# YamaneKoyo/mri-to-speech

Measured on AMD Instinct MI355X. Metric: rtMRI frames/s end-to-end (256x256 frames -> 64-bin mel -> 11413 Hz wav), higher is better.
Workload: dtype bf16x3; 1 GPU; e2e rtMRI->wav, 64 clips x 30 frames per GPU at 256x256 (configs[3] per-GPU share); clips_per_gpu=64, frames_per_clip=30, global_batch_clips=64, hw=256, parallelism=dp1, chunk=1920

## Files before the change

mri-to-speech_amd/csrc/conv1d_halo.hip:

```cpp
#include <cstring>

#include "conv_igemm.hpp"
#include "kernels.hpp"
#include "prof.hpp"

namespace m2s {
namespace {

__device__ __attribute__((aligned(16))) uint4 g_h1_zero[4];

constexpr int H1_BM = 128;
constexpr int H1_HIST = 64;
constexpr int H1_ROWS = H1_BM + H1_HIST;
constexpr int H1_PLANE = H1_ROWS * 16;

template <int C>
constexpr int h1_stage() {
  return 2 * (C / 16) * 1024;
}
template <int C>
constexpr int h1_slots() {
  return C <= 64 ? 4 : 3;
}
template <int C>
// ... 134 lines not shown
    for (int nt = 0; nt < NTW; ++nt) {
      const int n4 = (ntb + nt) * 16 + 4 * g;
      const float4 bb = *reinterpret_cast<const float4*>(a.bias + n4);
      float v[4] = {acc[i][nt][0] + bb.x, acc[i][nt][1] + bb.y, acc[i][nt][2] + bb.z, acc[i][nt][3] + bb.w};
      auto apply_act = [&]() {
        if (a.act == ACT_LRELU) {
#pragma unroll
          for (int j = 0; j < 4; ++j) v[j] = v[j] > 0.f ? v[j] : v[j] * a.act_slope;
        }
      };
      if (!a.act_after_res) apply_act();
      if (Rs) {
        float r[4], rl[4];
        unpack_bf16x4(prh[i][nt], r);
        unpack_bf16x4(prl[i][nt], rl);
#pragma unroll
        for (int j = 0; j < 4; ++j) {
          r[j] += rl[j];
          if (a.res_unslope != 0.f) r[j] = r[j] > 0.f ? r[j] : r[j] * a.res_unslope;
          v[j] += r[j];
        }
      }
      if (a.accum) {
        float p[4], pl[4];
        unpack_bf16x4(pyh[i][nt], p);
        unpack_bf16x4(pyl[i][nt], pl);
#pragma unroll
        for (int j = 0; j < 4; ++j) v[j] = (p[j] + pl[j]) + v[j];
        if (a.accum == 2) {
#pragma unroll
          for (int j = 0; j < 4; ++j) v[j] = v[j] / a.accum_div;
        }
      }
      if (a.act_after_res) apply_act();
      uint2 hi, lo;
      split4(v, hi, lo);
      *reinterpret_cast<uint2*>(Y + orow + n4) = hi;
      *reinterpret_cast<uint2*>(Y + orow + a.cs_out + n4) = lo;
    }
  }
}

template <int C>
void launch_c(const ConvBatch& b, int n, int B, int L, hipStream_t s, double flops, double bytes) {
  allow_lds(reinterpret_cast<const void*>(&conv1d_halo_sp_kernel<C>));
  const int tiles = ceil_div(L, H1_BM);
  char name[48];
  snprintf(name, sizeof(name), "conv1d_halo_sp_kernel<%d>", C);
  ProfScope ps(name, flops, bytes, s);
  hipLaunchKernelGGL((conv1d_halo_sp_kernel<C>), dim3(B * tiles, 1, n), dim3(64 * h1_waves<C>()), h1_lds<C>(), s, b, tiles);
  M2S_HIP(hipGetLastError());
}

}

bool conv1d_halo_sp_supported(int C, int cs, int k, int dil) {
  return C == 64 && cs == C && k >= 1 && k <= 31 && dil >= 1 && (k - 1) * dil <= H1_HIST;
}
size_t conv1d_halo_frag_elems(int C, int k) { return (size_t)k * (C / 32) * 2 * C * 32; }

void launch_conv1d_halo_sp(const ConvArgs* as, int n, hipStream_t s, double flops, double bytes) {
  M2S_CHECK(n >= 1 && n <= CONV_BATCH, "conv1d_halo: 1..CONV_BATCH convs");
  const ConvArgs& a = as[0];
  ConvBatch b;
  std::memset(&b, 0, sizeof(b));
  for (int i = 0; i < n; ++i) {
    const ConvArgs& c = as[i];
    M2S_CHECK(c.kind == KIND_CONV1D && c.cs_in == a.cs_in && c.cs_out == a.cs_in && c.M == a.M && c.L_in == c.L_out &&
                  c.L_out == a.L_out && c.in_xform == IN_NONE && c.pad_left == (c.ntaps - 1) * c.dil &&
                  conv1d_halo_sp_supported(a.cs_in, c.cs_in, c.ntaps, c.dil),
              "conv1d_halo: causal 1-D convs of one shape, C = 64, (k - 1) d <= 64");
    M2S_CHECK(c.x && c.w && c.bias && c.y && c.y != c.x && c.y != c.res, "conv1d_halo: operand pointers");
    for (int j = 0; j < i; ++j) M2S_CHECK(as[j].y != c.y, "conv1d_halo: two convs write one output");
    b.a[i] = c;
  }
  const int L = a.L_out, B = a.M / L;
  M2S_CHECK(B * L == a.M && L > 0, "conv1d_halo: M = clips x L");
  M2S_CHECK((double)a.M * a.cs_in * 2 < 2147483647.0, "conv1d_halo: 32-bit offsets");
  launch_c<64>(b, n, B, L, s, flops, bytes);
}

}
```

mri-to-speech_amd/csrc/kernels.hpp:

```cpp
#pragma once

#include "m2s_common.hpp"

namespace m2s {

enum AsyncCode : unsigned { M2S_ASYNC_LSTM = 1u, M2S_ASYNC_WS = 2u };
struct AsyncReport {
  unsigned spin_max = 1u << 20;
  unsigned* err = nullptr;
};
__device__ __forceinline__ void report_async(unsigned* err, unsigned code, int lane) {
  if (err && lane == 0) __hip_atomic_store(err, code, __ATOMIC_RELAXED, __HIP_MEMORY_SCOPE_SYSTEM);
}

template <typename T>
void launch_stem(const float* frames, int N, int H, int W, int OH, int OW, int pad_t, int pad_l,
                 const float* w9, const float* bias, int cout, int cs_out, T* y, hipStream_t s);

int dw_pixel_blocks(int OH, int OW);
template <typename T>
void launch_dwconv(const T* x, int N, int IH, int IW, int OH, int OW, int stride, int pad_t, int pad_l,
                   int C, int cs, const float* w9, const float* bias, T* y, float* sums, hipStream_t s);

template <typename T>
void launch_se_mean(const float* psum, int N, int npb, int cs, float inv_count, T* mean, hipStream_t s);

bool ir_fused_supported(int OH, int OW, int cs_in, int cs_mid, bool split);
void launch_ir_pwdw(const void* x, int N, int cs_in, int kp, const void* wpw, const float* bpw, const void* wdw,
                    const float* bdw, int OH, int OW, int cs_mid, void* y, void* se_mean, bool split, double flops,
                    double bytes, hipStream_t s, bool f8_out = false, const void* x8 = nullptr,
                    const void* w8 = nullptr, const float* wsc = nullptr, int kp8 = 0);
void launch_rows_e4m3(const void* x, long rows, int cs, void* y8, int ld8, hipStream_t s);

bool se_gemm_f8_supported(int P, int cs_in, int cs_out);
void launch_se_gemm_f8(const void* x8, int M, int P, int cs_in, const void* w8, int kp, int n_pad, const float* wscale,
                       const float* bias, const void* gate, const void* res, void* y, int cs_out, hipStream_t s,
                       double flops, double bytes, void* y8 = nullptr, int ld8 = 0);

bool se_gemm_sp_supported(int P, int cs_in, int cs_out);
void launch_se_gemm_sp(const void* x, int M, int P, int cs_in, const void* w, int n_pad, const float* bias,
                       const void* gate, const void* res, void* y, int cs_out, hipStream_t s, double flops, double bytes);

bool se_ws_supported(int P, int cs_in, int cs_out);
void launch_se_ws(const void* x, int M, int P, int cs_in, const void* w, int n_pad, const float* bias, const void* gate,
                  const void* res, void* y, int cs_out, hipStream_t s, double flops, double bytes, AsyncReport rep = {},
                  bool x_f32 = false);

bool se_ws_f8_supported(int P, int cs_in, int cs_out);
void launch_se_ws_f8(const void* x8, int M, int P, int cs_in, const void* w8, int kp, int n_pad, const float* wscale,
                     const float* bias, const void* gate, const void* res, void* y, int cs_out, hipStream_t s, double flops,
                     double bytes, void* y8 = nullptr, int ld8 = 0, AsyncReport rep = {});

bool ir_ws_supported(int H, int W, int cs_in, int kp, int cs_mid);
bool ir_ws_s2_supported(int H, int W, int cs_in, int kp, int cs_mid, int OH, int OW, int pad_t, int pad_l);
void launch_ir_ws(const void* x, int N, int H, int W, int cs_in, int kp, int cs_mid, const void* wpw, const float* bpw,
                  const float* wdw, const float* bdw, void* y, void* se_mean, double flops, double bytes,
                  hipStream_t s, AsyncReport rep = {}, int stride = 1, int OH = 0, int OW = 0, int pad_t = 0,
                  int pad_l = 0, double spill = 0.0, bool fm32 = false);
int ir_s2band_bands(int OH);
bool ir_s2band_supported(int IH, int IW, int OH, int OW, int cs_in, int kp, int cs_mid);
void launch_ir_s2band(const void* x, int N, int IH, int IW, int cs_in, int kp, const void* wpw, const float* bpw,
                      const float* wdw, const float* bdw, int OH, int OW, int pad_t, int pad_l, int cs_mid, void* y,
                      float* psum, bool split, double flops, double bytes, hipStream_t s, bool f8_out = false);
bool ir_fused_s2_supported(int IH, int IW, int cs_in, int cs_mid, bool split);
void launch_ir_pwdw_s2(const void* x, int N, int cs_in, int kp, const void* wpw, const float* bpw, const void* wdw,
                       const float* bdw, int IH, int IW, int OH, int OW, int pad_t, int pad_l, int cs_mid, void* y,
                       void* se_mean, bool split, double flops, double bytes, hipStream_t s, bool f8_out = false,
                       const void* x8 = nullptr, const void* w8 = nullptr, const float* wsc = nullptr, int kp8 = 0);

bool conv1d_halo_sp_supported(int C, int cs, int k, int dil);
size_t conv1d_halo_frag_elems(int C, int k);
void launch_conv1d_halo_sp(const struct ConvArgs* a, int n, hipStream_t s, double flops, double bytes);
bool rb1_fused_supported(int C, int cs, int k, const int* dil, int np, int kp, bool split);
int rb1_frag_taps(int C, int k, bool split);
void launch_rb1_fused(const bf16_t* x, bf16_t* s, int B, int L, int C, int k, int np, const int* dil,
                      const bf16_t* const* w1, const float* const* b1, const bf16_t* const* w2,
                      const float* const* b2, int kp, int accum, float div, bool split, double flops, double bytes,
                      hipStream_t st);

void launch_stem_b0(const float* frames, int N, int H, int W, int OH, int OW, int pad_t, int pad_l, const float* w9,
                    const float* b9, const void* w0, const float* b0, int kp0, const void* w1, const float* b1,
                    int kp1, void* y, bool split, double flops, double bytes, hipStream_t s);

bool se_excite_supported(int rd, int kp2, int cs_mid);
void launch_se_excite(const void* mean, int N, int mid, int cs_mid, const void* w1, int kp1, const float* b1,
                      int rd, const void* w2, int kp2, const float* b2, void* gate, bool split, hipStream_t s);

bool er_fused_supported(int H, int W, int cin, int mid, int cout, int kp_exp, int kp_pwl);
void launch_er_fused(const bf16_t* x, int N, int H, int W, const bf16_t* wexp, const float* bexp, const bf16_t* wpwl,
                     const float* bpwl, bf16_t* y, double flops, double bytes, hipStream_t s);

bool er8_fused_supported(int H, int W, int cin, int mid, int cout);
void launch_er8_fused(const bf16_t* x, int N, int H, int W, const uint8_t* wexp, const float* sexp, const float* bexp,
                      const uint8_t* wpwl, const float* spwl, const float* bpwl, bf16_t* y, double flops, double bytes,
                      hipStream_t s, const uint8_t* x8 = nullptr, uint8_t* y8 = nullptr);

bool er2_fused_supported(int H, int W, int cs_in, int mid, int cout, int kp_exp, int kp_pwl);
int er2_stage_elems();
bool er8w_fused_supported(int H, int W, int cs_in, int mid, int cout);
size_t er8w_stream_bytes();
void launch_er8w_fused(const bf16_t* x, const uint8_t* x8, int N, int H, int W, const uint8_t* wst, const float* sexp,
                       const float* bexp, const float* spwl, const float* bpwl, bf16_t* y, uint8_t* y8, double flops,
                       double bytes, hipStream_t s);
void launch_er2_fused(const bf16_t* x, int N, int H, int W, const bf16_t* wst, const float* bexp, const float* bpwl,
                      bf16_t* y, double flops, double bytes, hipStream_t s);

bool er_sp_supported(int H, int W, int cs_in, int mid, int cs_out);
int er_sp_nt_stages(int cs_in, int mid, int cs_out, int* nt);
void launch_er_sp(const void* x, int N, int H, int W, int cs_in, int mid, int cs_out, const void* wst, const float* bexp,
                  const float* bpwl, void* y, double flops, double bytes, hipStream_t s, bool merged = true);

bool ers2_fused_supported(int OH, int OW, int cs_in, int mid, int cs_out, int kp_exp, int kp_pwl);
int ers2_exp_elems(int cs_in, int mid);
bool ers2_sp_supported(int OH, int OW, int cs_in, int mid, int cs_out);
void launch_ers2_sp(const void* x, int N, int H, int W, int OH, int OW, int pad_t, int pad_l, int cs_in, int mid,
                    int cs_out, const void* wexp, const float* bexp, const void* wpwl, const float* bpwl, void* y,
                    double flops, double bytes, hipStream_t s);
void launch_ers2_fused(const bf16_t* x, int N, int H, int W, int OH, int OW, int pad_t, int pad_l, int cs_in, int mid,
                       int cs_out, const bf16_t* wexp, const float* bexp, const bf16_t* wpwl, const float* bpwl,
                       bf16_t* y, double flops, double bytes, hipStream_t s, uint8_t* y8 = nullptr);

void launch_preprocess(const uint8_t* frames, int N, int H, int W, int channels, float* out, hipStream_t s);

template <typename T>
void launch_gap(const T* x, int N, int P, int C, int cs, float* feats, hipStream_t s);
// ... 78 lines not shown
```

mri-to-speech_amd/csrc/model.cpp:

```cpp
#include "model.hpp"

#include <algorithm>
#include <cmath>
#include <cstdlib>
#include <cstring>
#include <initializer_list>
#include <type_traits>
#include <utility>

#include "pack.hpp"
#include "prof.hpp"

namespace m2s {

void Arena::upload(int device) {
  M2S_HIP(hipSetDevice(device));
  M2S_HIP(hipMalloc(&dev_, host_.size() + 256));
  M2S_HIP(hipMemcpy(dev_, host_.data(), host_.size(), hipMemcpyHostToDevice));
  std::vector<uint8_t>().swap(host_);
}

Arena::~Arena() {
  if (dev_) (void)hipFree(dev_);
}
// ... 742 lines not shown
  a.y = b.pre;
  a.M = (int)N;
  a.kwave = 0;
  run_conv<float>(a, p_.lstm_ih, s);
  {
    ProfScope ps("lstm_window_table_kernel", 0.0, 4.0 * (5.0 * B + 2.0 * S), s);
    launch_lstm_window_table(b.tab, B, W, p.mean, p.max_windows, b.win, s);
  }
  const size_t plane = (size_t)S * H;
  {
    const double cells = p.active[0] + (p.mean ? 0.0 : (double)S);
    ProfScope ps("lstm_window_step0_kernel", 0.0, 4.0 * cells * H * (3.0 + 2.0), s);
    launch_lstm_window_step0(b.pre, b.win, S, !p.mean, split, b.hop[0], b.c, p.mean ? b.hf : (W == 1 ? b.hm : nullptr),
                             p.mean ? b.hf + (size_t)W * plane : b.hm + (size_t)p.R * H, s);
  }
  const float* wperm = static_cast<const float*>(arena_.ptr(p_.whh_win));
  for (int j = 1; j < W; ++j) {
    const void* hin = b.hop[(j - 1) & 1];
    void* hout = j + 1 < W ? b.hop[j & 1] : nullptr;
    float* hf = p.mean ? b.hf + (size_t)j * plane : (j == W - 1 ? b.hm : nullptr);
    ProfScope ps(split ? "lstm_window_step_kernel<split>" : "lstm_window_step_kernel<f32>",
                 (split ? 3.0 : 2.0) * 4.0 * H * H * p.active[j], 4.0 * dirs * 4 * H * H + 4.0 * p.active[j] * H * 8.0, s);
    launch_lstm_window_step(b.pre, wperm, b.win, S, j, dirs, split, hin, hout, b.c, hf, (long)((size_t)W * plane), s);
  }
  if (p.mean) {
    double contrib = 0.0;
    for (int j = 0; j < W; ++j) contrib += p.active[j];
    ProfScope ps("lstm_window_mean_kernel", contrib * H, 4.0 * H * (contrib + 2.0 * p.N), s);
    launch_lstm_window_mean(b.hf, b.tab, B, W, S, p.N, p.max_len, b.hm, s);
  }
  if (mel_norm) {
    StageTag head("head");
    ProfScope ps("mel_head_kernel", 2.0 * p.R * H * n_mels_, 4.0 * p.R * (2 * H + n_mels_), s);
    launch_mel_head(b.hm, (int)p.R, H, static_cast<const float*>(arena_.ptr(p_.head_wt)),
                    static_cast<const float*>(arena_.ptr(p_.head_b)), n_mels_, mel_norm, s);
  }
  if (y) launch_add2(b.hm, b.hm + (size_t)p.R * H, y, (long)((size_t)p.R * H), s);
}

void Acoustic::forward_windowed(const float* frames, const int* lengths, const int* context, int B, long N, int H,
                                int W, int window, int merge, float* mel_norm, Workspace& ws, hipStream_t s) {
  M2S_CHECK(lstm_window_supported(hidden_), "windowed: rnn_hidden must be 640");
  window_plan(lengths, context, B, N, window, merge);
  ragged_check_stream(s);
  float* feats = feats_buf(ws, (size_t)N);
  effnet(frames, (int)N, H, W, feats, -1, nullptr, nullptr, ws, s);
  bilstm_windowed(feats, lengths, context, B, N, window, merge, nullptr, mel_norm, ws, s);
}

Vocoder::Vocoder(const StateDict& sd, const m2s_hifigan_h& h, int dtype, int device)
    : h_(h), dtype_(dtype), device_(device) {
  for (auto [name, v] : std::initializer_list<std::pair<const char*, bool*>>{
           {"M2S_MRF_FUSED", &mrf_fused_}, {"M2S_MRF_BATCH", &mrf_batch_}, {"M2S_MRF_HALO", &mrf_halo_},
           {"M2S_F8_MRF64", &f8_mrf64_},   {"M2S_F8_MRF32", &f8_mrf32_}})
    env_flag(name, *v);
  pack_vocoder(sd, h, dtype, f8_mrf64_, f8_mrf32_, arena_, p_);
  arena_.upload(device);
  p_.pre.resolve(arena_);
  for (auto& u : p_.ups) u.resolve(arena_);
  for (auto& rb : p_.rbs) {
    for (auto& c : rb.c1) c.resolve(arena_);
    for (auto& c : rb.c2) c.resolve(arena_);
    for (size_t o : rb.f1_off) rb.f1.push_back(static_cast<const bf16_t*>(arena_.ptr(o)));
    for (size_t o : rb.f2_off) rb.f2.push_back(static_cast<const bf16_t*>(arena_.ptr(o)));
    for (size_t o : rb.h1_off) rb.h1.push_back(static_cast<const bf16_t*>(arena_.ptr(o)));
    for (size_t o : rb.h2_off) rb.h2.push_back(static_cast<const bf16_t*>(arena_.ptr(o)));
    for (auto* qv : {&rb.q1, &rb.q2})
      for (RB::F8& f : *qv) {
        f.wp = arena_.ptr(f.w);
        f.sp = static_cast<const float*>(arena_.ptr(f.s));
        f.bp = static_cast<const float*>(arena_.ptr(f.b));
      }
  }
}

size_t Vocoder::act_elems(int B, int T) const {
  size_t m = (size_t)B * T * chan_stride(h_.upsample_initial_channel);
  size_t L = T;
  for (int i = 0; i < h_.n_up; ++i) {
    L *= h_.upsample_rates[i];
    m = std::max(m, (size_t)B * L * chan_stride(h_.upsample_initial_channel >> (i + 1)));
  }
  return m;
}

void* Vocoder::mel_in(Workspace& ws, int B, int T) const {
  return ws.take<char>((size_t)B * T * chan_stride(h_.num_mels) * act_bytes(dtype_));
}

template <typename T>
Vocoder::GenBufs<T> Vocoder::gen_bufs(Workspace& ws, int B, int T_) const {
  const size_t n = act_elems(B, T_) * Elem<T>::R;
  GenBufs<T> g{};
  g.X = ws.take<T>(n);
  for (T*& h : g.Hb) h = ws.take<T>(n);
  g.T1 = ws.take<T>(n);
  g.S = ws.take<T>(n);
  if (dtype_ == M2S_DT_FP8) g.E8 = ws.take<T>(n);
  if (std::is_same<T, sp_t>::value)
    for (auto& bt : g.Bt)
      for (T*& q : bt) q = ws.take<T>(n);
  return g;
}

void Vocoder::gen_ws(Workspace& ws, int B, int T) const {
  dispatch_act(dtype_, [&](auto t) { gen_bufs<typename decltype(t)::type>(ws, B, T); });
}

size_t Vocoder::workspace_bytes(int B, int T) const {
// ... 134 lines not shown
}


size_t Vocoder::chunk_workspace_bytes(const int* lengths, const int* context, const int* hold, int B) const {
  long n = 0;
  for (int b = 0; lengths && b < B; ++b) n += lengths[b];
  const ChunkPlan p = chunk_plan(lengths, context, hold, B, n);
  return Workspace::bytes([&](Workspace& ws) {
    ragged_bufs(ws, B, p.d.Tmax, 5 + h_.n_up);
    gen_ws(ws, B, p.d.Tmax);
  });
}

void Vocoder::forward_chunk(const float* mel, const int* lengths, const int* context, const int* hold, int B, long N,
                            float* wav, Workspace& ws, hipStream_t s) {
  const ChunkPlan p = chunk_plan(lengths, context, hold, B, N);
  const int nm = h_.num_mels, cs = chan_stride(nm), T = p.d.Tmax;
  const RaggedBufs cb = ragged_bufs(ws, B, T, 5 + h_.n_up);
  rtab_.upload_ints(p.tab.data(), p.tab.size(), cb.tab, s);
  Cone cone{};
  for (int l = 0; l < h_.n_up; ++l) {
    cone.drop[l] = p.drop[l];
    cone.keep[l] = p.keep[l];
    cone.mask[l] = p.mask ? cb.tab + (size_t)(4 + l) * B : nullptr;
  }
  dispatch_act(dtype_, [&](auto t) {
    using A = typename decltype(t)::type;
    {
      StageTag tag("glue");
      ProfScope ps(tname<A>("ragged_glue_kernel"), 0.0, 4.0 * N * nm * 2, s);
      launch_ragged_glue<A>(mel, cb.tab, B, T, nm, nullptr, nullptr, nullptr, nullptr, static_cast<A*>(cb.ln_buf), cs,
                            s);
    }
    run_t<A>(cb.ln_buf, B, T, cb.wav_pad, ws, s, p.mask ? cb.tab : nullptr, p.crop ? &cone : nullptr);
  });
  StageTag tag("voc_post");
  ProfScope ps("chunk_wav_pack_kernel", 0.0, 2.0 * 4.0 * p.out_rows * p_.hop, s);
  const int* const emit = cb.tab + (size_t)2 * B;
  launch_chunk_wav_pack(cb.wav_pad, emit, emit + B, emit + (size_t)2 * B, B, p.t_final, p_.hop, wav, s);
}

constexpr int CONV_POST_TAPS = 7;

template <typename T>
void Vocoder::mrf_stage_batched(int i, const T* X, T* S, T* const (*Bt)[3], int B, int L, bool act_out,
                                hipStream_t s) {
  const int nk = h_.n_kernels, np = (int)p_.rbs[i * nk].dil.size();
  int ord[CONV_BATCH];
  for (int j = 0; j < nk; ++j) ord[j] = j;
  std::sort(ord, ord + nk, [&](int x, int y) { return p_.rbs[i * nk + x].c1[0].kp > p_.rbs[i * nk + y].c1[0].kp; });
  auto a_in = [&](int j, int p) -> const T* { return p == 0 ? X : Bt[j][1 + ((p - 1) & 1)]; };
  bool halo = mrf_halo_;
  for (int j = 0; j < nk; ++j) halo = halo && !p_.rbs[i * nk + j].h1.empty();
  auto launch_batch = [&](ConvArgs* cs, int n, double fl, double by) {
    if (halo)
      launch_conv1d_halo_sp(cs, n, s, fl, by);
    else
      launch_conv_gemm_batch(cs, n, s, fl, by);
  };
  for (int p = 0; p < np; ++p) {
    ConvArgs cs[CONV_BATCH];
    double fl = 0.0, by = 0.0, f, b;
    for (int jj = 0; jj < nk; ++jj) {
      const int j = ord[jj];
      const RB& rb = p_.rbs[i * nk + j];
      ConvArgs c = conv_args(rb.c1[p]);
      if (halo) c.w = rb.h1[p];
      c.x = a_in(j, p);
      c.y = Bt[j][0];
      c.L_in = c.L_out = L;
      c.M = B * L;
      c.act = ACT_LRELU;
      c.act_slope = 0.1f;
      conv_cost<T>(c, rb.c1[p], &f, &b);
      fl += f;
      by += b;
      cs[jj] = c;
    }
    launch_batch(cs, nk, fl, by);
    fl = by = 0.0;
    for (int jj = 0; jj < nk; ++jj) {
      const int j = p + 1 < np ? ord[jj] : jj;
      const RB& rb = p_.rbs[i * nk + j];
      ConvArgs c = conv_args(rb.c2[p]);
      if (halo) c.w = rb.h2[p];
      c.x = Bt[j][0];
      c.res = a_in(j, p);
      c.res_unslope = 10.f;
      c.L_in = c.L_out = L;
      c.M = B * L;
      if (p + 1 < np) {
        c.y = Bt[j][1 + (p & 1)];
        c.act = ACT_LRELU;
        c.act_slope = 0.1f;
        c.act_after_res = 1;
        conv_cost<T>(c, rb.c2[p], &f, &b);
        fl += f;
        by += b;
        cs[jj] = c;
      } else {
        c.y = S;
        c.accum = j == 0 ? 0 : (j == nk - 1 ? 2 : 1);
        c.accum_div = (float)nk;
        if (act_out && j == nk - 1) {
          c.act = ACT_LRELU;
          c.act_slope = 0.1f;
// ... 225 lines not shown
```

mri-to-speech_amd/csrc/model.hpp:

```cpp
#pragma once

#include <map>
#include <string>
#include <vector>

#include "../../include/m2s.h"
#include "conv_igemm.hpp"
#include "kernels.hpp"

namespace m2s {

struct HostTensor {
  const float* data = nullptr;
  std::vector<int64_t> shape;
  size_t numel() const {
    size_t n = 1;
    for (auto d : shape) n *= (size_t)d;
    return n;
  }
};
using StateDict = std::map<std::string, HostTensor>;
StateDict make_state_dict(const m2s_tensor* t, int n);

class Arena {
// ... 119 lines not shown
  bool er_frag = false;
  size_t er8_wexp = 0, er8_sexp = 0, er8_wpwl = 0, er8_spwl = 0;
  bool er8 = false;
  size_t er8w_w = 0, er8w_sexp = 0, er8w_spwl = 0;
  bool er8w = false;
  size_t er_sp_w = 0;
  bool er_sp = false;
  bool ers_sp = false;
  size_t f8_w = 0, f8_s = 0, f8_b = 0;
  int f8_kp = 0, f8_npad = 0;
  bool f8_pwl = false;
  size_t f8x_w = 0, f8x_s = 0;
  int f8x_kp = 0;
  bool f8_pw = false;
};

struct AcousticPlan {
  size_t stem_w = 0, stem_b = 0;
  std::vector<Block> blocks;
  PConv lstm_ih;
  size_t whh = 0, head_wt = 0, head_b = 0;
  size_t whh_win = 0;
  int max_mid_cs = 0;
};
void pack_acoustic(const StateDict& sd, int n_mels, int hidden, int dtype, Arena& ar, AcousticPlan& p);

struct RB {
  int k = 3;
  std::vector<int> dil;
  std::vector<PConv> c1, c2;
  std::vector<size_t> f1_off, f2_off;
  std::vector<const bf16_t*> f1, f2;
  std::vector<size_t> h1_off, h2_off;
  std::vector<const bf16_t*> h1, h2;
  struct F8 {
    size_t w = 0, s = 0, b = 0;
    const void* wp = nullptr;
    const float* sp = nullptr;
    const float* bp = nullptr;
  };
  std::vector<F8> q1, q2;
};

struct VocoderPlan {
  PConv pre;
  std::vector<PConv> ups;
  std::vector<RB> rbs;
  size_t post_w = 0;
  float post_b = 0.f;
  int post_c = 0, hop = 1;
  int back = 0, ahead = 0, lvl_back[8] = {}, lvl_ahead[8] = {};
};
void pack_vocoder(const StateDict& sd, const m2s_hifigan_h& h, int dtype, bool f8_mrf64, bool f8_mrf32, Arena& ar,
                  VocoderPlan& p);

class Acoustic {
 public:
  Acoustic(const StateDict& sd, int n_mels, int hidden, int dtype, int device);
  ~Acoustic();
  Acoustic(const Acoustic&) = delete;
  Acoustic& operator=(const Acoustic&) = delete;
  unsigned take_async_error();
  unsigned lstm_spin_max_ = LSTM_SPIN_MAX;
  unsigned ws_spin_max_ = 1u << 20;
  AsyncReport ws_report() const {
    AsyncReport r;
    r.spin_max = ws_spin_max_;
    r.err = err_dev_;
    return r;
  }
  int device() const { return device_; }
  int n_mels() const { return n_mels_; }
  int chunk = 1920;
  bool ir_fused_ = true;
  bool ir_ws_ = true;
  bool ir_ws_s2_ = true;
  int irws_min_ = 512;
  bool irws_f32_ = true;
  int sews_min_cus_ = 1;
  bool stem_fused_ = true;
  bool f8_er_ = true;
  bool se_y8_ = true;
  bool f8_er2_ = true;
  bool er8_x8_ = true;
  bool f8_expand_ = true;
  bool f8_s2_ = true;
  bool se_fused_ = true;
  bool er_fused_ = true;
  bool se_sp_ = false;
  bool se_ws_ = true;
  bool er_mrg_ = true;
  bool ir_s2band_ = true;
  bool lstm_persistent_ = true;
  bool lstm_mid_ = true;
  bool lstm_x3_ = true;
  bool lstm_x3g_ = true;

  size_t workspace_bytes(int B, int T, int H, int W) const;
  void forward(const float* frames, int B, int T, int H, int W, float* mel_norm, Workspace& ws, hipStream_t s);
  void effnet(const float* frames, int N, int H, int W, float* feats, int stop_after, float* probe, int* probe_dims,
              Workspace& ws, hipStream_t s);
  void bilstm(const float* feats, int B, int T, float* y, float* mel_norm, Workspace& ws, hipStream_t s);
  size_t ragged_workspace_bytes(const int* lengths, int B, int H, int W) const;
  void bilstm_ragged(const float* feats, const int* lengths, int B, long N, float* y, float* mel_norm, Workspace& ws,
                     hipStream_t s);
  void forward_ragged(const float* frames, const int* lengths, int B, long N, int H, int W, float* mel_norm,
                      Workspace& ws, hipStream_t s);
// ... 47 lines not shown
  static size_t lstm_sync_bytes();
  RaggedTable rtab_;
  template <typename T>
  void effnet_t(const float* frames, int N, int H, int W, float* feats, int stop_after, float* probe, int* probe_dims,
                Workspace& ws, hipStream_t s);
  template <typename T>
  void effnet_cn(EffPass<T>& p, size_t k);
  template <typename T>
  void effnet_er(EffPass<T>& p, size_t k);
  template <typename T>
  void effnet_ir_front(EffPass<T>& p, size_t k);
  template <typename T>
  void effnet_ir_se(EffPass<T>& p, size_t k);
  template <typename T>
  void effnet_ir_pwl(EffPass<T>& p, size_t k);
  int pass_frames(int N) const;
  size_t effnet_x8(int H, int W) const;
  void effnet_dims(int H, int W, size_t* io_elems, size_t* mid_elems, size_t* se_elems) const;

  int dtype_, device_, n_mels_, hidden_;
  Arena arena_;
  AcousticPlan p_;
  unsigned* err_host_ = nullptr;
  unsigned* err_dev_ = nullptr;
  void* gsync_ = nullptr;
  unsigned gsync_epoch_ = 0;
};

class Vocoder {
 public:
  Vocoder(const StateDict& sd, const m2s_hifigan_h& h, int dtype, int device);
  int device() const { return device_; }
  int hop() const { return p_.hop; }
  int num_mels() const { return h_.num_mels; }
  size_t workspace_bytes(int B, int T) const;
  void forward(const float* mel, int layout, int B, int T, float* wav, Workspace& ws, hipStream_t s);
  void forward_from_norm(const float* mel_norm, const float* mean, const float* std_, int B, int T, float* mel_db,
                         float* mel_log, void* ln_buf, float* wav, Workspace& ws, hipStream_t s);
  size_t ragged_workspace_bytes(const int* lengths, int B) const;
  void forward_ragged(const float* mel, const int* lengths, int B, long N, float* wav, Workspace& ws, hipStream_t s);
  void forward_from_norm_ragged(const float* mel_norm, const float* mean, const float* std_, const int* lengths, int B,
                                long N, float* mel_db, float* mel_log, float* wav, Workspace& ws, hipStream_t s);
  void reach(int* back, int* ahead) const {
    *back = p_.back;
    *ahead = p_.ahead;
  }
  size_t chunk_workspace_bytes(const int* lengths, const int* context, const int* hold, int B) const;
  void forward_chunk(const float* mel, const int* lengths, const int* context, const int* hold, int B, long N,
                     float* wav, Workspace& ws, hipStream_t s);
  bool chunk_cone_ = true;
  size_t act_elems(int B, int T) const;
  bool mrf_fused_ = true;
  bool mrf_halo_ = true;
  bool f8_mrf64_ = false;
  bool f8_mrf32_ = false;
  bool mrf_batch_ = true;

 private:
  struct Cone {
    int drop[8], keep[8];
    const int* mask[8];
  };
  template <typename T>
  void run_t(const void* mel_nlc, int B, int Tn, float* wav, Workspace& ws, hipStream_t s, const int* tab = nullptr,
             const Cone* cone = nullptr);
  template <typename T>
  struct GenBufs {
    T *X, *Hb[2], *T1, *S;
    T* E8;
    T* Bt[CONV_BATCH][3];
  };
  template <typename T>
  GenBufs<T> gen_bufs(Workspace& ws, int B, int T_) const;
  void gen_ws(Workspace& ws, int B, int T) const;
  void* mel_in(Workspace& ws, int B, int T) const;
  struct RaggedBufs {
    int* tab;
    void* ln_buf;
    float* wav_pad;
  };
  RaggedBufs ragged_bufs(Workspace& ws, int B, int Tmax, int tab_cols = 2) const;
  struct ChunkPlan {
    RaggedDims d;
    long out_rows = 0;
    bool crop = false, mask = false;
    int drop[8] = {}, keep[8] = {};
    int t_final = 0;
    std::vector<int> tab;
  };
  ChunkPlan chunk_plan(const int* lengths, const int* context, const int* hold, int B, long rows) const;
  void ragged_run(const float* x, const float* mean, const float* std_, const int* lengths, int B, long N,
                  float* mel_db, float* mel_log, float* wav, Workspace& ws, hipStream_t s);
  template <typename T>
  void mrf_stage_batched(int i, const T* X, T* S, T* const (*Bt)[3], int B, int L, bool act_out, hipStream_t s);
  m2s_hifigan_h h_;
  int dtype_, device_;
  Arena arena_;
  VocoderPlan p_;
  RaggedTable rtab_;
};

struct PipelineBufs {
  float* mn;
  void* ln_t;
  char* rest;
  size_t rest_bytes;
// ... 7 lines not shown
```

mri-to-speech_amd/csrc/pack_vocoder.cpp:

```cpp
#include <algorithm>
#include <cmath>

#include "pack.hpp"

namespace m2s {

namespace {

std::vector<float> fold_wn(const StateDict& sd, const std::string& p, std::vector<int64_t> shape) {
  auto it = sd.find(p + ".weight");
  if (it != sd.end()) {
    const HostTensor& t = need(sd, p + ".weight", shape);
    return std::vector<float>(t.data, t.data + t.numel());
  }
  std::vector<int64_t> gs(shape.size(), 1);
  gs[0] = shape[0];
  const HostTensor& g = need(sd, p + ".weight_g", gs);
  const HostTensor& v = need(sd, p + ".weight_v", shape);
  const size_t inner = v.numel() / shape[0];
  std::vector<float> w(v.numel());
  for (int64_t i = 0; i < shape[0]; ++i) {
    double acc = 0.0;
    for (size_t j = 0; j < inner; ++j) acc += (double)v.data[i * inner + j] * v.data[i * inner + j];
    const float sc = g.data[i] / (float)std::sqrt(acc);
// ... 10 lines not shown
  int C, k;
  auto tap(int t) const {
    return [this, t](int n, int c) { return t < k ? wv[((size_t)n * C + c) * k + t] : 0.f; };
  }
};

size_t pack_rb1_frag(Arena& ar, const RbWeights& w, bool split) {
  const int taps = rb1_frag_taps(w.C, w.k, split), nt16 = w.C / 16, k32 = w.C / 32, planes = split ? 2 : 1;
  std::vector<uint16_t> f((size_t)taps * planes * nt16 * k32 * kFrag);
  size_t o = 0;
  for (int t = 0; t < taps; ++t)
    for (int pl = 0; pl < planes; ++pl)
      for (int nt = 0; nt < nt16; ++nt)
        for (int kc = 0; kc < k32; ++kc, o += kFrag)
          frag_bf16(&f[o], !split ? Plane::bf16 : pl == 0 ? Plane::hi : Plane::lo, nt, kc, w.tap(t));
  return ar.add_vec(f);
}

size_t pack_conv1d_halo(Arena& ar, const RbWeights& w) {
  std::vector<uint16_t> f(conv1d_halo_frag_elems(w.C, w.k));
  size_t o = 0;
  for (int t = 0; t < w.k; ++t)
    for (int kc = 0; kc < w.C / 32; ++kc)
      for (int pl = 0; pl < 2; ++pl)
        for (int nt = 0; nt < w.C / 16; ++nt, o += kFrag) frag_bf16(&f[o], pl == 0 ? Plane::hi : Plane::lo, nt, kc, w.tap(t));
  return ar.add_vec(f);
}

void generator_reach(const m2s_hifigan_h& h, VocoderPlan& p) {
  auto fdiv = [](long a, long b) { return a >= 0 ? a / b : -((-a + b - 1) / b); };
  long lo = 0, hi = p.hop - 1 + 6, scale = p.hop;
  for (int i = h.n_up - 1; i >= 0; --i) {
    long mrf = 0;
    for (int j = 0; j < h.n_kernels; ++j) {
      long r = 0;
      for (int d = 0; d < h.n_dilations[j]; ++d)
        r += (long)(h.resblock_kernel_sizes[j] - 1) * (h.resblock_dilation_sizes[j][d] + (h.resblock == 1 ? 1 : 0));
      mrf = std::max(mrf, r);
    }
    const long u = h.upsample_rates[i], k = h.upsample_kernel_sizes[i], pad = (k - u) / 2;
    lo = -fdiv(-(lo - mrf + pad - k + 1), u);
    hi = fdiv(hi + pad, u);
    scale /= u;
    p.lvl_back[i] = (int)-fdiv(lo, scale);
    p.lvl_ahead[i] = (int)fdiv(hi, scale);
  }
  p.back = (int)-lo;
  p.ahead = (int)hi + 6;
}

}

void pack_vocoder(const StateDict& sd, const m2s_hifigan_h& h, int dtype, bool f8_mrf64, bool f8_mrf32, Arena& ar,
                  VocoderPlan& p) {
  M2S_CHECK(dtype == M2S_DT_F32 || dtype == M2S_DT_BF16 || dtype == M2S_DT_BF16X3 || dtype == M2S_DT_FP8, "bad dtype");
  M2S_CHECK(h.resblock == 1 || h.resblock == 2, "resblock must be 1 or 2");
  const int io_dt = dtype == M2S_DT_FP8 ? M2S_DT_BF16 : dtype;
  M2S_CHECK(h.n_up >= 1 && h.n_up <= 8 && h.n_kernels >= 1 && h.n_kernels <= 8, "bad generator config");
  const int c0 = h.upsample_initial_channel;
  {
    const HostTensor& w = need(sd, "conv_pre.weight", {c0, h.num_mels, 7});
    const HostTensor& b = need(sd, "conv_pre.bias", {c0});
    p.pre = make_pconv(KIND_CONV1D, h.num_mels, c0, 7, io_dt);
    p.pre.ks = 7;
    p.pre.pad_left = 0;
    p.pre.macs_per_row = (double)c0 * h.num_mels * 7;
    const int ci = h.num_mels;
    pack_conv(ar, io_dt, p.pre, [&](int, int n, int t, int c) { return w.data[((size_t)n * ci + c) * 7 + t]; },
              [&](int n) { return b.data[n]; });
  }
  p.hop = 1;
  for (int i = 0; i < h.n_up; ++i) {
    const int u = h.upsample_rates[i], k = h.upsample_kernel_sizes[i];
    const int ci = c0 >> i, co = c0 >> (i + 1);
    M2S_CHECK(co >= 4, "generator too narrow");
    M2S_CHECK(u >= 1 && k >= u && (k - u) % 2 == 0,
              "upsample kernel " + std::to_string(k) + " / rate " + std::to_string(u) +
                  ": k - u must be even and >= 0 (output length L*u)");
    p.hop *= u;
    const std::string up = "ups." + std::to_string(i);
    std::vector<float> w = fold_wn(sd, up, {ci, co, k});
    const HostTensor& b = need(sd, up + ".bias", {co});
    PConv pc = make_pconv(KIND_CONVT, ci, co, (k + u - 1) / u, io_dt);
    pc.phases = u;
    pc.ct_u = u;
    pc.ct_pad = (k - u) / 2;
    pc.ct_k = k;
    pc.macs_per_row = (double)ci * co * k / u;
    const int pad = pc.ct_pad;
    pack_conv(ar, io_dt, pc,
              [&](int ph, int n, int t, int c) {
                const int j = (ph + pad) % u + t * u;
                return j < k ? w[((size_t)c * co + n) * k + j] : 0.f;
              },
              [&](int n) { return b.data[n]; });
    p.ups.push_back(pc);
    for (int j = 0; j < h.n_kernels; ++j) {
      RB rb;
      rb.k = h.resblock_kernel_sizes[j];
      const int kk = rb.k;
      M2S_CHECK(h.n_dilations[j] >= 1 && h.n_dilations[j] <= 8, "resblock dilations: 1..8 per kernel size");
      for (int d = 0; d < h.n_dilations[j]; ++d) rb.dil.push_back(h.resblock_dilation_sizes[j][d]);
      const std::string q = "resblocks." + std::to_string(i * h.n_kernels + j);
      const bool fsplit = dtype == M2S_DT_BF16X3;
      const bool frag = (dtype == M2S_DT_BF16 || dtype == M2S_DT_FP8 || fsplit) && h.resblock == 1 &&
                        rb1_fused_supported(co, chan_stride(co), kk, rb.dil.data(), (int)rb.dil.size(), kk * co, fsplit);
      const bool q8 = dtype == M2S_DT_FP8 && h.resblock == 1 &&
                      ((co >= 128 && !frag) || (co == 64 && f8_mrf64) || (co == 32 && f8_mrf32)) &&
                      conv1d_f8_supported(co, kk);
      bool halo = fsplit && h.resblock == 1 && !frag;
      for (size_t d = 0; d < rb.dil.size(); ++d) halo = halo && conv1d_halo_sp_supported(co, chan_stride(co), kk, rb.dil[d]);
      auto load = [&](const std::string& name) {
        return RbWeights{fold_wn(sd, name, {co, co, kk}), need(sd, name + ".bias", {co}).data, co, kk};
      };
      auto dense = [&](const RbWeights& w, int dil) {
        PConv c = make_pconv(KIND_CONV1D, co, co, kk, dtype);
        c.ks = kk;
        c.dil = dil;
        c.pad_left = (kk - 1) * dil;
        c.macs_per_row = (double)co * co * kk;
        pack_conv(ar, dtype, c, [&](int, int n, int t, int cc) { return w.wv[((size_t)n * co + cc) * kk + t]; },
                  [&](int n) { return w.bias[n]; });
        return c;
      };
      auto e4m3 = [&](const RbWeights& w) {
        RB::F8 f;
        pack_gemm_f8(
            ar, kk * co, co, co, round_up(kk * co, 128),
            [&](int n, int kx) { return w.wv[((size_t)n * co + kx % co) * kk + kx / co]; },
            [&](int n) { return w.bias[n]; }, &f.w, &f.s, &f.b);
        return f;
      };
      for (size_t d = 0; d < rb.dil.size(); ++d) {
        if (h.resblock == 2) {
          rb.c1.push_back(dense(load(q + ".convs." + std::to_string(d)), rb.dil[d]));
          continue;
        }
        const RbWeights w1 = load(q + ".convs1." + std::to_string(d));
        rb.c1.push_back(dense(w1, rb.dil[d]));
        const RbWeights w2 = load(q + ".convs2." + std::to_string(d));
        rb.c2.push_back(dense(w2, 1));
        if (frag) {
          rb.f1_off.push_back(pack_rb1_frag(ar, w1, fsplit));
          rb.f2_off.push_back(pack_rb1_frag(ar, w2, fsplit));
        }
        if (halo) {
          rb.h1_off.push_back(pack_conv1d_halo(ar, w1));
          rb.h2_off.push_back(pack_conv1d_halo(ar, w2));
        }
        if (q8) {
          rb.q1.push_back(e4m3(w1));
          rb.q2.push_back(e4m3(w2));
        }
      }
      p.rbs.push_back(rb);
    }
  }
  p.post_c = c0 >> h.n_up;
  {
    std::vector<float> w = fold_wn(sd, "conv_post", {1, p.post_c, 7});
    const HostTensor& b = need(sd, "conv_post.bias", {1});
    std::vector<float> wt((size_t)7 * p.post_c);
    for (int c = 0; c < p.post_c; ++c)
      for (int t = 0; t < 7; ++t) wt[(size_t)t * p.post_c + c] = w[(size_t)c * 7 + t];
// ... 8 lines not shown
```

Before: 50480 rtMRI frames/s.

## Fuse HiFi-GAN resblock conv pairs into one halo kernel with chained accumulation

Adds a conv1d_halo_pair kernel that computes both dilated and unit convs of a resblock-1 layer inside one tile. The intermediate activation stays in LDS, and the tile recomputes a 16-row halo so no second launch or global round trip is needed. A chain mode runs all kernel-size branches of the final dilation in one launch and keeps the running sum in registers, which removes the extra read-modify-write passes on the output. In exchange it recomputes the overlap rows and uses larger register and LDS state per block. The path is on by default for C=64 and behind a flag for C=128.

```diff
diff --git a/mri-to-speech_amd/csrc/conv1d_halo.hip b/mri-to-speech_amd/csrc/conv1d_halo.hip
--- a/mri-to-speech_amd/csrc/conv1d_halo.hip
+++ b/mri-to-speech_amd/csrc/conv1d_halo.hip
@@ -210,6 +210,290 @@
   M2S_HIP(hipGetLastError());
 }
 
+constexpr int H2_BM = 112;
+constexpr int H2_HALO = H1_BM - H2_BM;
+
+struct HaloPairBatch {
+  HaloPair p[CONV_BATCH];
+  int n, L, chain;
+  float div;
+};
+
+template <int C>
+__global__ void __launch_bounds__(64 * h1_waves<C>(), 2) conv1d_halo_pair_kernel(const HaloPairBatch pb, int tiles) {
+  constexpr int NPL = C / 8, NT = C / 16, KC = C / 32;
+  constexpr int NW = h1_waves<C>(), NTW = NT * 4 / NW;
+  constexpr int STAGE = h1_stage<C>();
+  constexpr int PPW = STAGE / 1024 / NW;
+  constexpr int SLOTS = h1_slots<C>();
+  extern __shared__ __attribute__((aligned(16))) char smem[];
+  char* img = smem;
+  char* ring = smem + 2 * NPL * H1_PLANE;
+
+  const int tid = threadIdx.x, lane = tid & 63;
+  const int wave = __builtin_amdgcn_readfirstlane(tid >> 6);
+  const int g = lane >> 4, r16 = lane & 15;
+  const int wr = wave & 3, ntb = (wave >> 2) * NTW;
+  const int clip = blockIdx.x / tiles, tile = blockIdx.x - clip * tiles;
+  const int L = pb.L, t0 = tile * H2_BM;
+  const char* zp = reinterpret_cast<const char*>(g_h1_zero);
+  asm volatile("" : "+s"(zp));
+  const uint32_t img0 = (uint32_t)(uintptr_t)img, ring0 = (uint32_t)(uintptr_t)ring;
+  const int njobs = pb.chain ? pb.n : 1;
+
+  float sum[2][NTW][4];
+#pragma unroll
+  for (int i = 0; i < 2; ++i)
+#pragma unroll
+    for (int nt = 0; nt < NTW; ++nt)
+#pragma unroll
+      for (int j = 0; j < 4; ++j) sum[i][nt][j] = 0.f;
+
+  for (int job = 0; job < njobs; ++job) {
+    const HaloPair a = pb.p[pb.chain ? job : (int)blockIdx.z];
+    const int Q1 = a.k * KC, Q = 2 * Q1;
+    const bf16_t* __restrict__ X = static_cast<const bf16_t*>(a.x);
+    const char* W1 = static_cast<const char*>(a.w1);
+    const char* W2 = static_cast<const char*>(a.w2);
+    bf16_t* __restrict__ Y = static_cast<bf16_t*>(a.y);
+    if (job) {
+      asm volatile("s_waitcnt lgkmcnt(0)" ::: "memory");
+      __builtin_amdgcn_s_barrier();
+      asm volatile("" ::: "memory");
+    }
+
+    uint2 pyh[2][NTW], pyl[2][NTW];
+    float4 b1v[NTW], b2v[NTW];
+#pragma unroll
+    for (int nt = 0; nt < NTW; ++nt) {
+      const int n4 = (ntb + nt) * 16 + 4 * g;
+      b1v[nt] = *reinterpret_cast<const float4*>(a.b1 + n4);
+      b2v[nt] = *reinterpret_cast<const float4*>(a.b2 + n4);
+    }
+#pragma unroll
+    for (int i = 0; i < 2; ++i) {
+      const int r = 32 * wr + 16 * i + r16, t = t0 - H2_HALO + r;
+      const bool own = r >= H2_HALO && t < L;
+      const size_t orow = ((size_t)clip * L + (own ? t : 0)) * C * 2;
+#pragma unroll
+      for (int nt = 0; nt < NTW; ++nt) {
+        const int n4 = (ntb + nt) * 16 + 4 * g;
+        pyh[i][nt] = pyl[i][nt] = make_uint2(0u, 0u);
+        if (a.accum && !pb.chain && own) {
+          pyh[i][nt] = *reinterpret_cast<const uint2*>(Y + orow + n4);
+          pyl[i][nt] = *reinterpret_cast<const uint2*>(Y + orow + C + n4);
+        }
+      }
+    }
+
+    {
+      constexpr int PIECES = 2 * NPL * (H1_ROWS / 64);
+      const int t = t0 - H2_HALO - H1_HIST + lane;
+      for (int pc = wave; pc < PIECES; pc += NW) {
+        const int p = pc / (H1_ROWS / 64), rb = pc - p * (H1_ROWS / 64);
+        const int half = p / NPL, ch = p - half * NPL, tt = t + 64 * rb;
+        const void* src = tt >= 0 && tt < L
+                              ? static_cast<const void*>(X + ((size_t)clip * L + tt) * (2 * C) + half * C + ch * 8)
+                              : static_cast<const void*>(zp);
+        dma16(src, __builtin_amdgcn_readfirstlane(img0 + (uint32_t)(p * H1_PLANE + rb * 1024)));
+      }
+    }
+    auto issue = [&](int q) {
+      const char* base = q < Q1 ? W1 + (size_t)q * STAGE : W2 + (size_t)(q - Q1) * STAGE;
+      const char* src = base + (wave * PPW) * 1024 + lane * 16;
+      const uint32_t dst = ring0 + (uint32_t)((q % SLOTS) * STAGE + wave * PPW * 1024);
+#pragma unroll
+      for (int j = 0; j < PPW; ++j)
+        dma16(q < Q ? static_cast<const void*>(src + j * 1024) : static_cast<const void*>(zp), dst + j * 1024);
+    };
+#pragma unroll
+    for (int q = 0; q < SLOTS - 1; ++q) issue(q);
+
+    f32x4 acc[2][NTW];
+#pragma unroll
+    for (int i = 0; i < 2; ++i)
+#pragma unroll
+      for (int nt = 0; nt < NTW; ++nt) acc[i][nt] = f32x4{0.f, 0.f, 0.f, 0.f};
+    uint2 prh[2][NTW], prl[2][NTW];
+#pragma unroll
+    for (int i = 0; i < 2; ++i)
+#pragma unroll
+      for (int nt = 0; nt < NTW; ++nt) prh[i][nt] = prl[i][nt] = make_uint2(0u, 0u);
+
+    int tap = 0, kc = 0, dil = a.dil;
+    for (int q = 0; q < Q; ++q) {
+      if (q == Q1) {
+#pragma unroll
+        for (int i = 0; i < 2; ++i)
+#pragma unroll
+          for (int nt = 0; nt < NTW; ++nt) {
+            const int n4 = (ntb + nt) * 16 + 4 * g;
+            const char* p = img + (n4 >> 3) * H1_PLANE + (H1_HIST + 32 * wr + 16 * i + r16) * 16 + (n4 & 7) * 2;
+            prh[i][nt] = *reinterpret_cast<const uint2*>(p);
+            prl[i][nt] = *reinterpret_cast<const uint2*>(p + NPL * H1_PLANE);
+          }
+        asm volatile("s_waitcnt lgkmcnt(0)" ::: "memory");
+        __builtin_amdgcn_s_barrier();
+        asm volatile("" ::: "memory");
+#pragma unroll
+        for (int i = 0; i < 2; ++i) {
+          const int t = t0 - H2_HALO + 32 * wr + 16 * i + r16;
+          const bool live = t >= 0 && t < L;
+#pragma unroll
+          for (int nt = 0; nt < NTW; ++nt) {
+            const int n4 = (ntb + nt) * 16 + 4 * g;
+            const float4 bb = b1v[nt];
+            float v[4] = {acc[i][nt][0] + bb.x, acc[i][nt][1] + bb.y, acc[i][nt][2] + bb.z, acc[i][nt][3] + bb.w};
+#pragma unroll
+            for (int j = 0; j < 4; ++j) v[j] = v[j] > 0.f ? v[j] : v[j] * 0.1f;
+            uint2 hi, lo;
+            split4(v, hi, lo);
+            if (!live) hi = lo = make_uint2(0u, 0u);
+            char* p = img + (n4 >> 3) * H1_PLANE + (H1_HIST + 32 * wr + 16 * i + r16) * 16 + (n4 & 7) * 2;
+            *reinterpret_cast<uint2*>(p) = hi;
+            *reinterpret_cast<uint2*>(p + NPL * H1_PLANE) = lo;
+            acc[i][nt] = f32x4{0.f, 0.f, 0.f, 0.f};
+          }
+        }
+        asm volatile("s_waitcnt lgkmcnt(0)" ::: "memory");
+        tap = 0;
+        dil = 1;
+      }
+      wait_vm<(SLOTS - 2) * PPW>();
+      __builtin_amdgcn_s_barrier();
+      asm volatile("" ::: "memory");
+      issue(q + SLOTS - 1);
+      const char* ws = ring + (q % SLOTS) * STAGE + lane * 16;
+      bf16x8 wh[NTW], wl[NTW];
+#pragma unroll
+      for (int nt = 0; nt < NTW; ++nt) {
+        wh[nt] = *reinterpret_cast<const bf16x8*>(ws + (ntb + nt) * 1024);
+        wl[nt] = *reinterpret_cast<const bf16x8*>(ws + (NT + ntb + nt) * 1024);
+      }
+      const int shift = (a.k - 1 - tap) * dil;
+      const char* ib = img + (kc * 4 + g) * H1_PLANE + (H1_HIST + 32 * wr + r16 - shift) * 16;
+#pragma unroll
+      for (int i = 0; i < 2; ++i) {
+        const bf16x8 bh = *reinterpret_cast<const bf16x8*>(ib + i * 256);
+        const bf16x8 bl = *reinterpret_cast<const bf16x8*>(ib + NPL * H1_PLANE + i * 256);
+#pragma unroll
+        for (int nt = 0; nt < NTW; ++nt) {
+          acc[i][nt] = __builtin_amdgcn_mfma_f32_16x16x32_bf16(wl[nt], bh, acc[i][nt], 0, 0, 0);
+          acc[i][nt] = __builtin_amdgcn_mfma_f32_16x16x32_bf16(wh[nt], bl, acc[i][nt], 0, 0, 0);
+          acc[i][nt] = __builtin_amdgcn_mfma_f32_16x16x32_bf16(wh[nt], bh, acc[i][nt], 0, 0, 0);
+        }
+      }
+      if (++kc == KC) {
+        kc = 0;
+        ++tap;
+      }
+    }
+    wait_vm<0>();
+
+    const bool keep = pb.chain && job + 1 < njobs;
+#pragma unroll
+    for (int i = 0; i < 2; ++i) {
+      const int r = 32 * wr + 16 * i + r16, t = t0 - H2_HALO + r;
+      if (r < H2_HALO || t >= L) continue;
+      const size_t orow = ((size_t)clip * L + t) * C * 2;
+#pragma unroll
+      for (int nt = 0; nt < NTW; ++nt) {
+        const int n4 = (ntb + nt) * 16 + 4 * g;
+        const float4 bb = b2v[nt];
+        float v[4] = {acc[i][nt][0] + bb.x, acc[i][nt][1] + bb.y, acc[i][nt][2] + bb.z, acc[i][nt][3] + bb.w};
+        float rr[4], rl[4];
+        unpack_bf16x4(prh[i][nt], rr);
+        unpack_bf16x4(prl[i][nt], rl);
+#pragma unroll
+        for (int j = 0; j < 4; ++j) {
+          rr[j] += rl[j];
+          rr[j] = rr[j] > 0.f ? rr[j] : rr[j] * 10.f;
+          v[j] += rr[j];
+        }
+        if (a.accum) {
+          float p[4], pl[4];
+          unpack_bf16x4(pyh[i][nt], p);
+          unpack_bf16x4(pyl[i][nt], pl);
+#pragma unroll
+          for (int j = 0; j < 4; ++j) v[j] = (pb.chain ? sum[i][nt][j] : p[j] + pl[j]) + v[j];
+          if (a.accum == 2) {
+#pragma unroll
+            for (int j = 0; j < 4; ++j) v[j] = v[j] / pb.div;
+          }
+        }
+        if (a.act) {
+#pragma unroll
+          for (int j = 0; j < 4; ++j) v[j] = v[j] > 0.f ? v[j] : v[j] * 0.1f;
+        }
+        uint2 hi, lo;
+        split4(v, hi, lo);
+        if (keep) {
+          float h[4], l[4];
+          unpack_bf16x4(hi, h);
+          unpack_bf16x4(lo, l);
+#pragma unroll
+          for (int j = 0; j < 4; ++j) sum[i][nt][j] = h[j] + l[j];
+        } else {
+          *reinterpret_cast<uint2*>(Y + orow + n4) = hi;
+          *reinterpret_cast<uint2*>(Y + orow + C + n4) = lo;
+        }
+      }
+    }
+  }
+}
+
+}
+
+bool conv1d_halo_pair_supported(int C, int cs, int k, int dil) {
+  return (C == 64 || C == 128) && cs == C && k >= 1 && dil >= 1 && (k - 1) * dil + (k - 1) <= H1_HIST &&
+         k - 1 <= H2_HALO;
+}
+
+namespace {
+template <int C>
+bool pair_fills(int B, int L) {
+  const void* kern = reinterpret_cast<const void*>(&conv1d_halo_pair_kernel<C>);
+  allow_lds(kern);
+  return (long)B * ceil_div(L, H2_BM) >= device_resident(kern, 64 * h1_waves<C>(), h1_lds<C>());
+}
+template <int C>
+void launch_pair(const HaloPairBatch& b, int B, int tiles, hipStream_t s, double flops, double bytes) {
+  allow_lds(reinterpret_cast<const void*>(&conv1d_halo_pair_kernel<C>));
+  char name[48];
+  snprintf(name, sizeof(name), "conv1d_halo_pair_kernel<%d>", C);
+  ProfScope ps(name, flops, bytes, s);
+  hipLaunchKernelGGL((conv1d_halo_pair_kernel<C>), dim3(B * tiles, 1, b.chain ? 1 : b.n), dim3(64 * h1_waves<C>()),
+                     h1_lds<C>(), s, b, tiles);
+  M2S_HIP(hipGetLastError());
+}
+}
+
+bool conv1d_halo_pair_fills(int C, int B, int L) { return C == 64 ? pair_fills<64>(B, L) : C == 128 && pair_fills<128>(B, L); }
+
+void launch_conv1d_halo_pair(const HaloPair* ps, int n, int C, int B, int L, bool chain, float div, hipStream_t s,
+                             double flops, double bytes) {
+  M2S_CHECK(n >= 1 && n <= CONV_BATCH, "conv1d_halo pair: 1..CONV_BATCH pairs");
+  M2S_CHECK((C == 64 || C == 128) && B > 0 && L > 0, "conv1d_halo pair: C = 64 or 128");
+  M2S_CHECK((double)B * L * C * 2 < 2147483647.0, "conv1d_halo pair: 32-bit offsets");
+  HaloPairBatch b;
+  std::memset(&b, 0, sizeof(b));
+  for (int i = 0; i < n; ++i) {
+    const HaloPair& c = ps[i];
+    M2S_CHECK(conv1d_halo_pair_supported(C, C, c.k, c.dil), "conv1d_halo pair: (k - 1) d + (k - 1) <= 64, k <= 17");
+    M2S_CHECK(c.x && c.w1 && c.w2 && c.b1 && c.b2 && c.y, "conv1d_halo pair: operand pointers");
+    for (int j = 0; j < n; ++j) M2S_CHECK(ps[j].x != c.y, "conv1d_halo pair: an output is a pair's input");
+    for (int j = 0; j < i && !chain; ++j) M2S_CHECK(ps[j].y != c.y, "conv1d_halo pair: two pairs write one output");
+    b.p[i] = c;
+  }
+  b.n = n;
+  b.L = L;
+  b.chain = chain ? 1 : 0;
+  b.div = div;
+  const int tiles = ceil_div(L, H2_BM);
+  if (C == 64)
+    launch_pair<64>(b, B, tiles, s, flops, bytes);
+  else
+    launch_pair<128>(b, B, tiles, s, flops, bytes);
 }
 
 bool conv1d_halo_sp_supported(int C, int cs, int k, int dil) {
diff --git a/mri-to-speech_amd/csrc/kernels.hpp b/mri-to-speech_amd/csrc/kernels.hpp
--- a/mri-to-speech_amd/csrc/kernels.hpp
+++ b/mri-to-speech_amd/csrc/kernels.hpp
@@ -71,6 +71,21 @@
 bool conv1d_halo_sp_supported(int C, int cs, int k, int dil);
 size_t conv1d_halo_frag_elems(int C, int k);
 void launch_conv1d_halo_sp(const struct ConvArgs* a, int n, hipStream_t s, double flops, double bytes);
+struct HaloPair {
+  const void* x;
+  const void* w1;
+  const void* w2;
+  const float* b1;
+  const float* b2;
+  void* y;
+  int k, dil;
+  int accum;
+  int act;
+};
+bool conv1d_halo_pair_supported(int C, int cs, int k, int dil);
+bool conv1d_halo_pair_fills(int C, int B, int L);
+void launch_conv1d_halo_pair(const HaloPair* p, int n, int C, int B, int L, bool chain, float div, hipStream_t s,
+                             double flops, double bytes);
 bool rb1_fused_supported(int C, int cs, int k, const int* dil, int np, int kp, bool split);
 int rb1_frag_taps(int C, int k, bool split);
 void launch_rb1_fused(const bf16_t* x, bf16_t* s, int B, int L, int C, int k, int np, const int* dil,
diff --git a/mri-to-speech_amd/csrc/model.cpp b/mri-to-speech_amd/csrc/model.cpp
--- a/mri-to-speech_amd/csrc/model.cpp
+++ b/mri-to-speech_amd/csrc/model.cpp
@@ -818,9 +818,10 @@
     : h_(h), dtype_(dtype), device_(device) {
   for (auto [name, v] : std::initializer_list<std::pair<const char*, bool*>>{
            {"M2S_MRF_FUSED", &mrf_fused_}, {"M2S_MRF_BATCH", &mrf_batch_}, {"M2S_MRF_HALO", &mrf_halo_},
-           {"M2S_F8_MRF64", &f8_mrf64_},   {"M2S_F8_MRF32", &f8_mrf32_}})
+           {"M2S_F8_MRF64", &f8_mrf64_},   {"M2S_F8_MRF32", &f8_mrf32_},   {"M2S_MRF_PAIR", &mrf_pair_},
+           {"M2S_MRF_CHAIN", &mrf_chain_}, {"M2S_MRF_PAIR128", &mrf_pair128_}})
     env_flag(name, *v);
-  pack_vocoder(sd, h, dtype, f8_mrf64_, f8_mrf32_, arena_, p_);
+  pack_vocoder(sd, h, dtype, f8_mrf64_, f8_mrf32_, arena_, p_, mrf_pair_ && mrf_pair128_);
   arena_.upload(device);
   p_.pre.resolve(arena_);
   for (auto& u : p_.ups) u.resolve(arena_);
@@ -1061,6 +1062,55 @@
   auto a_in = [&](int j, int p) -> const T* { return p == 0 ? X : Bt[j][1 + ((p - 1) & 1)]; };
   bool halo = mrf_halo_;
   for (int j = 0; j < nk; ++j) halo = halo && !p_.rbs[i * nk + j].h1.empty();
+  const int C = p_.ups[i].cout;
+  bool pair = halo && mrf_pair_ && std::is_same<T, sp_t>::value && (C == 64 || mrf_pair128_);
+  for (int j = 0; j < nk && pair; ++j)
+    for (int d : p_.rbs[i * nk + j].dil) pair = pair && conv1d_halo_pair_supported(C, chan_stride(C), p_.rbs[i * nk + j].k, d);
+  for (int j = 0; j < nk; ++j)
+    for (int d : p_.rbs[i * nk + j].dil) halo = halo && conv1d_halo_sp_supported(C, chan_stride(C), p_.rbs[i * nk + j].k, d);
+  if (pair) {
+    const double es = sizeof(T) * Elem<T>::R, act = es * B * L * C;
+    auto make = [&](int j, int p, double* fl, double* by) {
+      const RB& rb = p_.rbs[i * nk + j];
+      HaloPair h{};
+      h.x = a_in(j, p);
+      h.w1 = rb.h1[p];
+      h.w2 = rb.h2[p];
+      h.b1 = conv_args(rb.c1[p]).bias;
+      h.b2 = conv_args(rb.c2[p]).bias;
+      h.k = rb.k;
+      h.dil = rb.dil[p];
+      *fl += 2.0 * (rb.c1[p].macs_per_row + rb.c2[p].macs_per_row) * B * L;
+      *by += act + es * 2.0 * C * C * rb.k;
+      return h;
+    };
+    for (int p = 0; p + 1 < np; ++p) {
+      HaloPair hp[CONV_BATCH];
+      double fl = 0.0, by = 0.0;
+      for (int jj = 0; jj < nk; ++jj) {
+        hp[jj] = make(ord[jj], p, &fl, &by);
+        hp[jj].y = Bt[ord[jj]][1 + (p & 1)];
+        hp[jj].act = 1;
+        by += act;
+      }
+      launch_conv1d_halo_pair(hp, nk, C, B, L, false, 1.f, s, fl, by);
+    }
+    HaloPair hp[CONV_BATCH];
+    double fl = 0.0, by = 0.0;
+    const bool chain = mrf_chain_ && conv1d_halo_pair_fills(C, B, L);
+    for (int j = 0; j < nk; ++j) {
+      double f = 0.0, b = 0.0;
+      hp[j] = make(j, np - 1, &f, &b);
+      hp[j].y = S;
+      hp[j].accum = j == 0 ? 0 : (j == nk - 1 ? 2 : 1);
+      hp[j].act = act_out && j == nk - 1;
+      if (!chain) launch_conv1d_halo_pair(&hp[j], 1, C, B, L, false, (float)nk, s, f, b + act * (hp[j].accum ? 2 : 1));
+      fl += f;
+      by += b;
+    }
+    if (chain) launch_conv1d_halo_pair(hp, nk, C, B, L, true, (float)nk, s, fl, by + act);
+    return;
+  }
   auto launch_batch = [&](ConvArgs* cs, int n, double fl, double by) {
     if (halo)
       launch_conv1d_halo_sp(cs, n, s, fl, by);
diff --git a/mri-to-speech_amd/csrc/model.hpp b/mri-to-speech_amd/csrc/model.hpp
--- a/mri-to-speech_amd/csrc/model.hpp
+++ b/mri-to-speech_amd/csrc/model.hpp
@@ -195,7 +195,7 @@
   int back = 0, ahead = 0, lvl_back[8] = {}, lvl_ahead[8] = {};
 };
 void pack_vocoder(const StateDict& sd, const m2s_hifigan_h& h, int dtype, bool f8_mrf64, bool f8_mrf32, Arena& ar,
-                  VocoderPlan& p);
+                  VocoderPlan& p, bool pair128 = false);
 
 class Acoustic {
  public:
@@ -349,6 +349,9 @@
   size_t act_elems(int B, int T) const;
   bool mrf_fused_ = true;
   bool mrf_halo_ = true;
+  bool mrf_pair_ = true;
+  bool mrf_chain_ = true;
+  bool mrf_pair128_ = false;
   bool f8_mrf64_ = false;
   bool f8_mrf32_ = false;
   bool mrf_batch_ = true;
diff --git a/mri-to-speech_amd/csrc/pack_vocoder.cpp b/mri-to-speech_amd/csrc/pack_vocoder.cpp
--- a/mri-to-speech_amd/csrc/pack_vocoder.cpp
+++ b/mri-to-speech_amd/csrc/pack_vocoder.cpp
@@ -86,7 +86,7 @@
 }
 
 void pack_vocoder(const StateDict& sd, const m2s_hifigan_h& h, int dtype, bool f8_mrf64, bool f8_mrf32, Arena& ar,
-                  VocoderPlan& p) {
+                  VocoderPlan& p, bool pair128) {
   M2S_CHECK(dtype == M2S_DT_F32 || dtype == M2S_DT_BF16 || dtype == M2S_DT_BF16X3 || dtype == M2S_DT_FP8, "bad dtype");
   M2S_CHECK(h.resblock == 1 || h.resblock == 2, "resblock must be 1 or 2");
   const int io_dt = dtype == M2S_DT_FP8 ? M2S_DT_BF16 : dtype;
@@ -143,7 +143,9 @@
                       ((co >= 128 && !frag) || (co == 64 && f8_mrf64) || (co == 32 && f8_mrf32)) &&
                       conv1d_f8_supported(co, kk);
       bool halo = fsplit && h.resblock == 1 && !frag;
-      for (size_t d = 0; d < rb.dil.size(); ++d) halo = halo && conv1d_halo_sp_supported(co, chan_stride(co), kk, rb.dil[d]);
+      for (size_t d = 0; d < rb.dil.size(); ++d)
+        halo = halo && (conv1d_halo_sp_supported(co, chan_stride(co), kk, rb.dil[d]) ||
+                        (pair128 && co == 128 && conv1d_halo_pair_supported(co, chan_stride(co), kk, rb.dil[d])));
       auto load = [&](const std::string& name) {
         return RbWeights{fold_wn(sd, name, {co, co, kk}), need(sd, name + ".bias", {co}).data, co, kk};
       };
```

Result: faster. 51120 rtMRI frames/s, median of 6 (+1.3%).
